# lbrndnr/LBAudioDetective

Measured on AMD Instinct MI355X. Metric: audio_seconds_fingerprinted_per_sec, higher is better.
Workload: dtype f32; 1 GPU; configs[1]: 100k synthetic 1 s @44.1 kHz mono clips, 1024-pt FFT, stride 64, fingerprint-only, input resident in HBM; one step = 13 passes over the batch; clips_per_gpu=100000, samples_per_clip=44100, window=1024, stride=64, bands=32, subfingerprints_per_clip=5, kernel_variant=0, parallelism=clips sharded x1, no collective

## Files before the change

### lbaudiodetective_amd/csrc/k_haar_select32.hip

```cpp
#include "internal.hpp"
#include "const_div.hpp"

#include <type_traits>

namespace lbad {
namespace {

constexpr uint32_t kCand = 128;
constexpr int kChunkDw = 20;


constexpr uint32_t kHistBuckets = 2048;

__device__ __forceinline__ uint32_t wave_prefix_sum(uint32_t x) {
    x += (uint32_t)__builtin_amdgcn_update_dpp(0, (int)x, 0x111 , 0xF, 0xF, false);
    x += (uint32_t)__builtin_amdgcn_update_dpp(0, (int)x, 0x112 , 0xF, 0xF, false);
    x += (uint32_t)__builtin_amdgcn_update_dpp(0, (int)x, 0x114 , 0xF, 0xF, false);
    x += (uint32_t)__builtin_amdgcn_update_dpp(0, (int)x, 0x118 , 0xF, 0xF, false);
    x += (uint32_t)__builtin_amdgcn_update_dpp(0, (int)x, 0x142 , 0xA, 0xF, false);
    x += (uint32_t)__builtin_amdgcn_update_dpp(0, (int)x, 0x143 , 0xC, 0xF, false);
    return x;
}

template <int WAVES>
__device__ __forceinline__ uint32_t slots_sum(const uint32_t* slot) {
    uint32_t c = 0;
#pragma unroll
    for (int w = 0; w < WAVES; ++w) c += slot[w];
    return c;
}

template <int WAVES>
__device__ __forceinline__ uint32_t block_sum(uint32_t v, uint32_t* s_red, int parity) {
#pragma unroll
    for (int off = 32; off > 0; off >>= 1) v += __shfl_xor(v, off, 64);
    uint32_t* slot = s_red + 8 * parity;
    if ((threadIdx.x & 63) == 0) slot[threadIdx.x >> 6] = v;
    __syncthreads();
    return slots_sum<WAVES>(slot);
}

constexpr uint32_t kLightLo = 0x25800000u;
typedef float f2 __attribute__((ext_vector_type(2)));

struct LightGuard {
    uint32_t lo_in = 0xFFFFFFFFu, lo_4 = 0xFFFFFFFFu;
    float hi = 0.0f;
    __device__ __forceinline__ void levels34(f2 a, f2 b, f2 c) {
        auto t = [](float x) { return (__float_as_uint(x) << 1) - 1u; };
        lo_4 = min(min(min(t(a.x), t(a.y)), min(t(b.x), t(b.y))), min(t(c.x), t(c.y)));
    }
    __device__ __forceinline__ bool bad(float s4) const {
        return lo_in < 2u * kLightLo - 1u || lo_4 < 2u * kFastDivLo - 1u || !(hi <= __uint_as_float(kFastDivHi)) || s4 != s4;
    }
};

template <bool FAST>
__device__ __forceinline__ float haar16_impl(const float (&in)[16], float (&d)[15], float root, float r_root,
                                             float root2, float r_root2, DivGuard& g) {
    float a[16];
#pragma unroll
    for (int i = 0; i < 16; i += 2) {
        if constexpr (FAST) {
            g.inputs(in[i], in[i + 1]);
            g.dividends(in[i], in[i + 1]);
        }
        a[i] = div_c<FAST>(in[i], root, r_root);
        a[i + 1] = div_c<FAST>(in[i + 1], root, r_root);
    }
    auto bfly = [&](float x, float y, float& sum, float& dif) {
        const float sp = __fadd_rn(x, y), sm = __fsub_rn(x, y);
        if constexpr (FAST) g.dividends(sp, sm);
        sum = div_c<FAST>(sp, root2, r_root2);
        dif = div_c<FAST>(sm, root2, r_root2);
    };
    float s1[8], s2[4], s3[2], s4;
#pragma unroll
    for (int i = 0; i < 8; ++i) bfly(a[2 * i], a[2 * i + 1], s1[i], d[i]);
#pragma unroll
    for (int i = 0; i < 4; ++i) bfly(s1[2 * i], s1[2 * i + 1], s2[i], d[8 + i]);
#pragma unroll
    for (int i = 0; i < 2; ++i) bfly(s2[2 * i], s2[2 * i + 1], s3[i], d[12 + i]);
    bfly(s3[0], s3[1], s4, d[14]);
    return s4;
}


struct DivConst {
    unsigned long long r, nd;
    __device__ __forceinline__ explicit DivConst(float d)
        : r(__builtin_amdgcn_readfirstlane(__float_as_uint(__fdiv_rn(1.0f, d)))),
          nd(__builtin_amdgcn_readfirstlane(__float_as_uint(-d))) {}
};

__device__ __forceinline__ void pk_prescale8(f2 (&x)[8], f2 (&q)[8], const DivConst& c) {
    asm("v_pk_mul_f32 %0, %8, %[r] op_sel_hi:[1,0]\n"
        "v_pk_mul_f32 %1, %9, %[r] op_sel_hi:[1,0]\n"
        "v_pk_mul_f32 %2, %10, %[r] op_sel_hi:[1,0]\n"
        "v_pk_mul_f32 %3, %11, %[r] op_sel_hi:[1,0]\n"
        "v_pk_mul_f32 %4, %12, %[r] op_sel_hi:[1,0]\n"
        "v_pk_mul_f32 %5, %13, %[r] op_sel_hi:[1,0]\n"
        "v_pk_mul_f32 %6, %14, %[r] op_sel_hi:[1,0]\n"
        "v_pk_mul_f32 %7, %15, %[r] op_sel_hi:[1,0]\n"
        "v_pk_fma_f32 %8, %0, %[nd], %8 op_sel_hi:[1,0,1]\n"
        "v_pk_fma_f32 %9, %1, %[nd], %9 op_sel_hi:[1,0,1]\n"
        "v_pk_fma_f32 %10, %2, %[nd], %10 op_sel_hi:[1,0,1]\n"
        "v_pk_fma_f32 %11, %3, %[nd], %11 op_sel_hi:[1,0,1]\n"
        "v_pk_fma_f32 %12, %4, %[nd], %12 op_sel_hi:[1,0,1]\n"
        "v_pk_fma_f32 %13, %5, %[nd], %13 op_sel_hi:[1,0,1]\n"
        "v_pk_fma_f32 %14, %6, %[nd], %14 op_sel_hi:[1,0,1]\n"
        "v_pk_fma_f32 %15, %7, %[nd], %15 op_sel_hi:[1,0,1]\n"
        "v_pk_fma_f32 %0, %8, %[r], %0 op_sel_hi:[1,0,1]\n"
        "v_pk_fma_f32 %1, %9, %[r], %1 op_sel_hi:[1,0,1]\n"
        "v_pk_fma_f32 %2, %10, %[r], %2 op_sel_hi:[1,0,1]\n"
        "v_pk_fma_f32 %3, %11, %[r], %3 op_sel_hi:[1,0,1]\n"
        "v_pk_fma_f32 %4, %12, %[r], %4 op_sel_hi:[1,0,1]\n"
        "v_pk_fma_f32 %5, %13, %[r], %5 op_sel_hi:[1,0,1]\n"
        "v_pk_fma_f32 %6, %14, %[r], %6 op_sel_hi:[1,0,1]\n"
        "v_pk_fma_f32 %7, %15, %[r], %7 op_sel_hi:[1,0,1]\n"
        "s_nop 0"
        : "=&v"(q[0]), "=&v"(q[1]), "=&v"(q[2]), "=&v"(q[3]), "=&v"(q[4]), "=&v"(q[5]), "=&v"(q[6]), "=&v"(q[7]),
          "+v"(x[0]), "+v"(x[1]), "+v"(x[2]), "+v"(x[3]), "+v"(x[4]), "+v"(x[5]), "+v"(x[6]), "+v"(x[7])
        : [r] "s"(c.r), [nd] "s"(c.nd));
}

__device__ __forceinline__ void pk_level1(f2 (&p)[8], f2 (&q)[8], const DivConst& c) {
    asm("v_pk_add_f32 %8, %8, %8 op_sel:[0,1] op_sel_hi:[0,1] neg_hi:[0,1]\n"
        "v_pk_add_f32 %9, %9, %9 op_sel:[0,1] op_sel_hi:[0,1] neg_hi:[0,1]\n"
        "v_pk_add_f32 %10, %10, %10 op_sel:[0,1] op_sel_hi:[0,1] neg_hi:[0,1]\n"
        "v_pk_add_f32 %11, %11, %11 op_sel:[0,1] op_sel_hi:[0,1] neg_hi:[0,1]\n"
        "v_pk_add_f32 %12, %12, %12 op_sel:[0,1] op_sel_hi:[0,1] neg_hi:[0,1]\n"
        "v_pk_add_f32 %13, %13, %13 op_sel:[0,1] op_sel_hi:[0,1] neg_hi:[0,1]\n"
        "v_pk_add_f32 %14, %14, %14 op_sel:[0,1] op_sel_hi:[0,1] neg_hi:[0,1]\n"
        "v_pk_add_f32 %15, %15, %15 op_sel:[0,1] op_sel_hi:[0,1] neg_hi:[0,1]\n"
        "v_pk_mul_f32 %0, %8, %[r] op_sel_hi:[1,0]\n"
        "v_pk_mul_f32 %1, %9, %[r] op_sel_hi:[1,0]\n"
        "v_pk_mul_f32 %2, %10, %[r] op_sel_hi:[1,0]\n"
        "v_pk_mul_f32 %3, %11, %[r] op_sel_hi:[1,0]\n"
        "v_pk_mul_f32 %4, %12, %[r] op_sel_hi:[1,0]\n"
        "v_pk_mul_f32 %5, %13, %[r] op_sel_hi:[1,0]\n"
        "v_pk_mul_f32 %6, %14, %[r] op_sel_hi:[1,0]\n"
        "v_pk_mul_f32 %7, %15, %[r] op_sel_hi:[1,0]\n"
        "v_pk_fma_f32 %8, %0, %[nd], %8 op_sel_hi:[1,0,1]\n"
        "v_pk_fma_f32 %9, %1, %[nd], %9 op_sel_hi:[1,0,1]\n"
        "v_pk_fma_f32 %10, %2, %[nd], %10 op_sel_hi:[1,0,1]\n"
        "v_pk_fma_f32 %11, %3, %[nd], %11 op_sel_hi:[1,0,1]\n"
        "v_pk_fma_f32 %12, %4, %[nd], %12 op_sel_hi:[1,0,1]\n"
        "v_pk_fma_f32 %13, %5, %[nd], %13 op_sel_hi:[1,0,1]\n"
        "v_pk_fma_f32 %14, %6, %[nd], %14 op_sel_hi:[1,0,1]\n"
        "v_pk_fma_f32 %15, %7, %[nd], %15 op_sel_hi:[1,0,1]\n"
        "v_pk_fma_f32 %0, %8, %[r], %0 op_sel_hi:[1,0,1]\n"
        "v_pk_fma_f32 %1, %9, %[r], %1 op_sel_hi:[1,0,1]\n"
        "v_pk_fma_f32 %2, %10, %[r], %2 op_sel_hi:[1,0,1]\n"
        "v_pk_fma_f32 %3, %11, %[r], %3 op_sel_hi:[1,0,1]\n"
        "v_pk_fma_f32 %4, %12, %[r], %4 op_sel_hi:[1,0,1]\n"
        "v_pk_fma_f32 %5, %13, %[r], %5 op_sel_hi:[1,0,1]\n"
        "v_pk_fma_f32 %6, %14, %[r], %6 op_sel_hi:[1,0,1]\n"
        "v_pk_fma_f32 %7, %15, %[r], %7 op_sel_hi:[1,0,1]\n"
        "s_nop 0"
        : "=&v"(q[0]), "=&v"(q[1]), "=&v"(q[2]), "=&v"(q[3]), "=&v"(q[4]), "=&v"(q[5]), "=&v"(q[6]), "=&v"(q[7]),
          "+v"(p[0]), "+v"(p[1]), "+v"(p[2]), "+v"(p[3]), "+v"(p[4]), "+v"(p[5]), "+v"(p[6]), "+v"(p[7])
        : [r] "s"(c.r), [nd] "s"(c.nd));
}

__device__ __forceinline__ void pk_level2(const f2 (&p)[8], f2 (&q)[4], const DivConst& c) {
    f2 t0, t1, t2, t3;
    asm("v_pk_add_f32 %4, %8, %9 op_sel:[0,0] op_sel_hi:[0,0] neg_hi:[0,1]\n"
        "v_pk_add_f32 %5, %10, %11 op_sel:[0,0] op_sel_hi:[0,0] neg_hi:[0,1]\n"
        "v_pk_add_f32 %6, %12, %13 op_sel:[0,0] op_sel_hi:[0,0] neg_hi:[0,1]\n"
        "v_pk_add_f32 %7, %14, %15 op_sel:[0,0] op_sel_hi:[0,0] neg_hi:[0,1]\n"
        "v_pk_mul_f32 %0, %4, %[r] op_sel_hi:[1,0]\n"
        "v_pk_mul_f32 %1, %5, %[r] op_sel_hi:[1,0]\n"
        "v_pk_mul_f32 %2, %6, %[r] op_sel_hi:[1,0]\n"
        "v_pk_mul_f32 %3, %7, %[r] op_sel_hi:[1,0]\n"
        "v_pk_fma_f32 %4, %0, %[nd], %4 op_sel_hi:[1,0,1]\n"
        "v_pk_fma_f32 %5, %1, %[nd], %5 op_sel_hi:[1,0,1]\n"
        "v_pk_fma_f32 %6, %2, %[nd], %6 op_sel_hi:[1,0,1]\n"
        "v_pk_fma_f32 %7, %3, %[nd], %7 op_sel_hi:[1,0,1]\n"
        "v_pk_fma_f32 %0, %4, %[r], %0 op_sel_hi:[1,0,1]\n"
        "v_pk_fma_f32 %1, %5, %[r], %1 op_sel_hi:[1,0,1]\n"
        "v_pk_fma_f32 %2, %6, %[r], %2 op_sel_hi:[1,0,1]\n"
        "v_pk_fma_f32 %3, %7, %[r], %3 op_sel_hi:[1,0,1]\n"
        "s_nop 0"
        : "=&v"(q[0]), "=&v"(q[1]), "=&v"(q[2]), "=&v"(q[3]), "=&v"(t0), "=&v"(t1), "=&v"(t2), "=&v"(t3)
        : "v"(p[0]), "v"(p[1]), "v"(p[2]), "v"(p[3]), "v"(p[4]), "v"(p[5]), "v"(p[6]), "v"(p[7]), [r] "s"(c.r), [nd] "s"(c.nd));
}

__device__ __forceinline__ void pk_level34(const f2 (&p)[4], f2 (&q3)[2], f2& q4, f2 (&s3)[2], f2& s4, const DivConst& c) {
    f2 e0, e1, e4;
    asm("v_pk_add_f32 %3, %9, %10 op_sel:[0,0] op_sel_hi:[0,0] neg_hi:[0,1]\n"
        "v_pk_add_f32 %4, %11, %12 op_sel:[0,0] op_sel_hi:[0,0] neg_hi:[0,1]\n"
        "v_pk_mul_f32 %0, %3, %[r] op_sel_hi:[1,0]\n"
        "v_pk_mul_f32 %1, %4, %[r] op_sel_hi:[1,0]\n"
        "v_pk_fma_f32 %6, %0, %[nd], %3 op_sel_hi:[1,0,1]\n"
        "v_pk_fma_f32 %7, %1, %[nd], %4 op_sel_hi:[1,0,1]\n"
        "v_pk_fma_f32 %0, %6, %[r], %0 op_sel_hi:[1,0,1]\n"
        "v_pk_fma_f32 %1, %7, %[r], %1 op_sel_hi:[1,0,1]\n"
        "s_nop 0\n"
        "v_pk_add_f32 %5, %0, %1 op_sel:[0,0] op_sel_hi:[0,0] neg_hi:[0,1]\n"
        "s_nop 0\n"
        "v_pk_mul_f32 %2, %5, %[r] op_sel_hi:[1,0]\n"
        "s_nop 0\n"
        "v_pk_fma_f32 %8, %2, %[nd], %5 op_sel_hi:[1,0,1]\n"
        "s_nop 0\n"
        "v_pk_fma_f32 %2, %8, %[r], %2 op_sel_hi:[1,0,1]\n"
        "s_nop 0"
        : "=&v"(q3[0]), "=&v"(q3[1]), "=&v"(q4), "=&v"(s3[0]), "=&v"(s3[1]), "=&v"(s4), "=&v"(e0), "=&v"(e1), "=&v"(e4)
        : "v"(p[0]), "v"(p[1]), "v"(p[2]), "v"(p[3]), [r] "s"(c.r), [nd] "s"(c.nd));
}

__device__ __forceinline__ float max3_abs(float m, float a, float b) {
    float o;
    asm("v_max3_f32 %0, %1, |%2|, |%3|" : "=v"(o) : "v"(m), "v"(a), "v"(b));
    return o;
}

template <typename Load>
__device__ __forceinline__ float haar16(Load load, float (&d)[15], float root, float root2, bool& fast) {
    const DivConst c_root(root), c_root2(root2);
    {
        f2 x[8], q[8], u[8], v2[4], w[2], z, s3[2], s4;
        {
            float in[16];
            load(in);
#pragma unroll
            for (int i = 0; i < 8; ++i) x[i] = f2{in[2 * i], in[2 * i + 1]};
        }
        LightGuard lg;
#pragma unroll
        for (int i = 0; i < 8; ++i) {
            lg.lo_in = min(lg.lo_in, min((__float_as_uint(x[i].x) << 1) - 1u, (__float_as_uint(x[i].y) << 1) - 1u));
            lg.hi = max3_abs(lg.hi, x[i].x, x[i].y);
        }
        pk_prescale8(x, q, c_root);
        pk_level1(q, u, c_root2);
        pk_level2(u, v2, c_root2);
        pk_level34(v2, w, z, s3, s4, c_root2);
        lg.levels34(s3[0], s3[1], s4);
        fast = !__any(lg.bad(z.x));
        if (fast) {
#pragma unroll
            for (int i = 0; i < 8; ++i) d[i] = u[i].y;
#pragma unroll
            for (int i = 0; i < 4; ++i) d[8 + i] = v2[i].y;
            d[12] = w[0].y; d[13] = w[1].y; d[14] = z.y;
            return z.x;
        }
    }
    asm volatile("" ::: "memory");
    float in[16];
    load(in);
    DivGuard g;
    float s4 = haar16_impl<true>(in, d, root, __fdiv_rn(1.0f, root), root2, __fdiv_rn(1.0f, root2), g);
    fast = !__any(g.bad());
    if (!fast) s4 = haar16_impl<false>(in, d, root, 0.0f, root2, 0.0f, g);
    return s4;
}

template <int M>
__device__ __forceinline__ float lane_xor(float x) {
    static_assert(M == 1 || M == 2 || M == 4, "lane distance");
    const int i = __float_as_int(x);
    if constexpr (M == 1) return __int_as_float(__builtin_amdgcn_mov_dpp(i, 0xB1, 0xF, 0xF, true));
    else if constexpr (M == 2) return __int_as_float(__builtin_amdgcn_mov_dpp(i, 0x4E, 0xF, 0xF, true));
    else return __int_as_float(__builtin_amdgcn_ds_swizzle(i, 0x101F));
}

template <bool FAST, int LANES, int M = 1>
__device__ __forceinline__ void cross_level_step(float& cur, float& fin, bool& done, int h, float root2, float r_root2, DivGuard& g) {
    if constexpr (M < LANES) {
        const float other = lane_xor<M>(cur);
        const bool upper = (h & M) != 0;
        const float lo = upper ? other : cur, hi = upper ? -cur : other;
        const float s = __fadd_rn(lo, hi);
        if constexpr (FAST) g.dividends(s, s);
        const float q = div_c<FAST>(s, root2, r_root2);
        if (!done && upper) { fin = q; done = true; }
        cur = q;
        cross_level_step<FAST, LANES, 2 * M>(cur, fin, done, h, root2, r_root2, g);
    }
}

template <bool FAST, int LANES>
__device__ __forceinline__ float cross_levels_impl(float cur, int h, float root2, float r_root2, DivGuard& g) {
    float fin = 0.0f;
    bool done = false;
    cross_level_step<FAST, LANES>(cur, fin, done, h, root2, r_root2, g);
    if (!done) fin = cur;
    return fin;
}

template <int LANES>
__device__ __forceinline__ float cross_levels(float cur, int h, float root2, bool fast) {
    if constexpr (LANES == 1) return cur;
    if (fast) {
        DivGuard g;
        const float fin = cross_levels_impl<true, LANES>(cur, h, root2, __fdiv_rn(1.0f, root2), g);
        if (!__any(g.bad())) return fin;
    }
    DivGuard g;
    return cross_levels_impl<false, LANES>(cur, h, root2, 0.0f, g);
}

struct SparseArgs {
    uint32_t left, n_cols;
    uint32_t row_dw;
    uint32_t pos_left;
    uint32_t pos_right[4];
    uint32_t cols[8];
    uint32_t rank[8];
};
constexpr int kSparseCols = 21;
__device__ __forceinline__ uint32_t byte_of(const uint32_t (&tbl)[8], uint32_t i) { return (tbl[i >> 2] >> (8u * (i & 3u))) & 0xFFu; }

constexpr uint32_t kRmask44k = 0xFFF5u;
typedef float f4u __attribute__((ext_vector_type(4), aligned(4)));
typedef float f3u __attribute__((ext_vector_type(3), aligned(4)));
typedef float f2u __attribute__((ext_vector_type(2), aligned(4)));

template <int COLS, bool SPARSE, uint32_t RMASK = 0u, bool HAS_LEFT = false>
__global__ __launch_bounds__(SPARSE ? 192 : COLS * 8, SPARSE ? 8 : COLS == 64 ? 6 : 7) void haar_select32_kernel(const float* __restrict__ frames, uint32_t keep,
                                                                          uint32_t subfp_len, uint32_t* __restrict__ packed,
                                                                          float* __restrict__ haar_out, const SparseArgs sp) {
    static_assert(!SPARSE || COLS == 32, "the sparse form is for 32 bands");
    constexpr int kCols = COLS;
    constexpr int kThreads = SPARSE ? 192 : COLS * 8;
    constexpr int kWavesPerWg = kThreads / 64;
    constexpr int H = COLS / 16;
    constexpr uint32_t kIdxBits = COLS == 16 ? 11 : COLS == 32 ? 12 : 13;
    __shared__ __attribute__((aligned(16))) float s_t[(SPARSE ? kSparseCols : kCols) * 8 * kChunkDw];
    __shared__ __attribute__((aligned(16))) unsigned long long s_cand[kCand];
    __shared__ uint32_t s_rank[kCand];
    __shared__ uint32_t s_red[16];
    __shared__ uint32_t s_ncand;
    __shared__ uint32_t s_bits[kPackedWords];
    __shared__ uint8_t s_pos[128];
    __shared__ uint32_t s_sel[4];
    static_assert(sizeof(s_t) >= kHistBuckets * sizeof(uint32_t), "the histogram lives in the transposed coefficients' LDS");

    const int t = threadIdx.x;
    const uint64_t frame = blockIdx.x;
    const float root2 = __fsqrt_rn(2.0f);
#ifdef LBAD_EXP_TIMELINE
    long long ts[8];
    int n_steps = 0;
#define STAMP(i) ts[i] = __builtin_readcyclecounter()
#define COUNT_STEP() ++n_steps
#else
#define STAMP(i)
#define COUNT_STEP()
#endif
    STAMP(0);

    float pre[16];
    float pre_left = 0.0f;
    auto fetch_row = [&](float (&a)[16], float& left_value) {
        if constexpr (SPARSE && RMASK != 0u) {
            constexpr int kRight = __builtin_popcount(RMASK), kRow = kRight + (HAS_LEFT ? 1 : 0);
            const bool mine = t < (int)kRowsPerFrame;
            const float* rowp = frames + frame * (kRowsPerFrame * kRow) + (mine ? t : 0) * kRow;
            float got[kRow + 3];
#pragma unroll
            for (int q = 0; q + 4 <= kRow; q += 4) {
                const f4u v = *reinterpret_cast<const f4u*>(rowp + q);
                got[q] = v.x; got[q + 1] = v.y; got[q + 2] = v.z; got[q + 3] = v.w;
            }
            constexpr int kDone = kRow & ~3;
            if constexpr (kRow - kDone == 3) {
                const f3u v = *reinterpret_cast<const f3u*>(rowp + kDone);
                got[kDone] = v.x; got[kDone + 1] = v.y; got[kDone + 2] = v.z;
            } else if constexpr (kRow - kDone == 2) {
                const f2u v = *reinterpret_cast<const f2u*>(rowp + kDone);
                got[kDone] = v.x; got[kDone + 1] = v.y;
            } else if constexpr (kRow - kDone == 1) {
                got[kDone] = rowp[kDone];
            }
#pragma unroll
            for (int jj = 0; jj < 16; ++jj)
                a[jj] = ((RMASK >> jj) & 1u) ? got[__builtin_popcount(RMASK & ((1u << jj) - 1u))] : 0.0f;
            left_value = HAS_LEFT ? got[kRight] : 0.0f;
        } else if constexpr (SPARSE) {
            const bool mine = t < (int)kRowsPerFrame;
            const float* rowp = frames + frame * (kRowsPerFrame * sp.row_dw) + (mine ? t : 0) * sp.row_dw;
            float got[16];
#pragma unroll
            for (int jj = 0; jj < 16; ++jj) {
                const uint32_t pos = (sp.pos_right[jj >> 2] >> (8 * (jj & 3))) & 0xFFu;
                got[jj] = rowp[pos != 0xFFu ? pos : 0u];
            }
            const float got_left = rowp[sp.left < 32u ? sp.pos_left : 0u];
#pragma unroll
            for (int jj = 0; jj < 16; ++jj) {
                const uint32_t pos = (sp.pos_right[jj >> 2] >> (8 * (jj & 3))) & 0xFFu;
                a[jj] = pos != 0xFFu ? got[jj] : 0.0f;
            }
            left_value = sp.left < 32u ? got_left : 0.0f;
        } else {
            const float4* src = reinterpret_cast<const float4*>(frames + frame * (kRowsPerFrame * kCols) + (t / H) * kCols + 16 * (t % H));
#pragma unroll
            for (int q = 0; q < 4; ++q) {
                const float4 v = src[q];
                a[4 * q] = v.x; a[4 * q + 1] = v.y; a[4 * q + 2] = v.z; a[4 * q + 3] = v.w;
            }
        }
    };
    fetch_row(pre, pre_left);
    bool first_read = true;

    if (t < (int)kPackedWords) s_bits[t] = 0;
    if (t < (int)kCand) s_rank[t] = 0;
    if (t == 0) s_ncand = 0;
    if (t < 128) {
        const int i = t >> 3, jj = t & 7;
        const int cross = (jj & 1) ? 4 + (jj >> 1) : (jj & 2) ? 2 + (jj >> 2) : (jj ? 1 : 0);
        s_pos[t] = (uint8_t)(i < 8 ? 64 + 8 * jj + i : i < 12 ? 32 + 4 * jj + (i - 8) : i < 14 ? 16 + 2 * jj + (i - 12) : i == 14 ? 8 + jj : cross);
    }
    for (int i = t; i < 2 * (int)kCand; i += kThreads)
        reinterpret_cast<uint32_t*>(s_cand)[i] = 0;

    if constexpr (SPARSE) {
        if (t < (int)kRowsPerFrame) {
            const int row = t;
            float d[15];
            auto load = [&](float (&a)[16]) {
                if (first_read) {
#pragma unroll
                    for (int jj = 0; jj < 16; ++jj) a[jj] = pre[jj];
                } else {
                    float again;
                    fetch_row(a, again);
                }
                first_read = false;
            };
            const float root = __fsqrt_rn(32.0f);
            bool fast;
            const float s4r = haar16(load, d, root, root2, fast);
            const float xl = pre_left;
            float det[4], s4l = 0.0f;
            auto chain = [&](auto fast_tag, DivGuard& g) {
                constexpr bool F = decltype(fast_tag)::value;
                const float r_root = F ? __fdiv_rn(1.0f, root) : 0.0f, r_root2 = F ? __fdiv_rn(1.0f, root2) : 0.0f;
                if constexpr (F) { g.inputs(xl, xl); g.dividends(xl, xl); }
                float a = div_c<F>(xl, root, r_root);
#pragma unroll
                for (int k = 0; k < 4; ++k) {
                    const bool odd = ((sp.left >> k) & 1u) != 0u;
                    const float sum_in = __fadd_rn(a, 0.0f);
                    if constexpr (F) g.dividends(sum_in, sum_in);
                    const float sum = div_c<F>(sum_in, root2, r_root2);
                    det[k] = odd ? -sum : sum;
                    a = sum;
                }
                s4l = a;
            };
            float avg = 0.0f, det5 = 0.0f;
            auto level5 = [&](auto fast_tag, DivGuard& g) {
                constexpr bool F = decltype(fast_tag)::value;
                const float r_root2 = F ? __fdiv_rn(1.0f, root2) : 0.0f;
                const float sp5 = __fadd_rn(s4l, s4r), sm5 = __fadd_rn(s4l, -s4r);
                if constexpr (F) g.dividends(sp5, sm5);
                avg = div_c<F>(sp5, root2, r_root2);
                det5 = div_c<F>(sm5, root2, r_root2);
            };
            {
                DivGuard g;
                chain(std::true_type{}, g);
                if (fast) level5(std::true_type{}, g);
                if (!fast || __any(g.bad())) {
                    chain(std::false_type{}, g);
                    level5(std::false_type{}, g);
                }
            }
            float* base = s_t + (row >> 4) * kChunkDw + (row & 15);
            auto put = [&](uint32_t pos, float value) {
                const uint32_t slot = byte_of(sp.rank, pos);
                if (slot != 0xFFu) base[slot * (8 * kChunkDw)] = value;
            };
#pragma unroll
            for (int i = 0; i < 8; ++i) put(24 + i, d[i]);
#pragma unroll
            for (int i = 0; i < 4; ++i) put(12 + i, d[8 + i]);
#pragma unroll
            for (int i = 0; i < 2; ++i) put(6 + i, d[12 + i]);
            put(3, d[14]);
            if (sp.left < 32u) {
                put(16 + (sp.left >> 1), det[0]);
                put(8 + (sp.left >> 2), det[1]);
                put(4 + (sp.left >> 3), det[2]);
                put(2, det[3]);
            }
            put(0, avg);
            put(1, det5);
        }
    } else
    {
        const int row = t / H, h = t % H;
        float d[15];
        auto load = [&](float (&a)[16]) {
            if (first_read) {
#pragma unroll
                for (int jj = 0; jj < 16; ++jj) a[jj] = pre[jj];
            } else {
                float unused;
                fetch_row(a, unused);
            }
            first_read = false;
        };
        bool fast;
        const float cur = haar16(load, d, __fsqrt_rn((float)kCols), root2, fast);
        const float fin = cross_levels<H>(cur, h, root2, fast);
        const int cross = H == 1 ? 0 : (h & 1) ? H / 2 + (h >> 1) : (h & 2) ? H / 4 + (h >> 2) : 0;
        float* base = s_t + (row >> 4) * kChunkDw + (row & 15);
#pragma unroll
        for (int i = 0; i < 8; ++i) base[(8 * H + 8 * h + i) * (8 * kChunkDw)] = d[i];
#pragma unroll
        for (int i = 0; i < 4; ++i) base[(4 * H + 4 * h + i) * (8 * kChunkDw)] = d[8 + i];
#pragma unroll
        for (int i = 0; i < 2; ++i) base[(2 * H + 2 * h + i) * (8 * kChunkDw)] = d[12 + i];
        base[(H + h) * (8 * kChunkDw)] = d[14];
        base[cross * (8 * kChunkDw)] = fin;
    }
    __syncthreads();
    STAMP(1);

    const bool live_thread = !SPARSE || (uint32_t)(t >> 3) < sp.n_cols;
    const bool live_wave = !SPARSE || (uint32_t)((t & ~63) >> 3) < sp.n_cols;
    const int cslot = SPARSE ? (live_thread ? t >> 3 : 0) : t >> 3;
    int col = t >> 3;
    if constexpr (SPARSE) col = (int)byte_of(sp.cols, (uint32_t)cslot);
    const int j = t & 7;
    float v[16];
    if (!live_wave) {
#pragma unroll
        for (int i = 0; i < 16; ++i) v[i] = 0.0f;
    } else {
        float d[15];
        const float4* src = reinterpret_cast<const float4*>(s_t + (cslot * 8 + j) * kChunkDw);
        auto load = [&](float (&a)[16]) {
#pragma unroll
            for (int q = 0; q < 4; ++q) {
                const float4 x = src[q];
                a[4 * q] = x.x; a[4 * q + 1] = x.y; a[4 * q + 2] = x.z; a[4 * q + 3] = x.w;
            }
        };
        bool fast;
        const float cur = haar16(load, d, __fsqrt_rn((float)kRowsPerFrame), root2, fast);
        const float fin = cross_levels<8>(cur, j, root2, fast);
#pragma unroll
        for (int i = 0; i < 8; ++i) v[i] = d[i];
#pragma unroll
        for (int i = 0; i < 4; ++i) v[8 + i] = d[8 + i];
        v[12] = d[12];
        v[13] = d[13];
        v[14] = d[14];
        v[15] = fin;
        if constexpr (SPARSE) {
            if (!live_thread) {
#pragma unroll
                for (int i = 0; i < 16; ++i) v[i] = 0.0f;
            }
        }
    }
    auto pos_of = [](int i, uint32_t jj) -> uint32_t {
        return i < 8 ? 64u + 8u * jj + (uint32_t)i : i < 12 ? 32u + 4u * jj + (uint32_t)(i - 8) : i < 14 ? 16u + 2u * jj + (uint32_t)(i - 12)
             : i == 14 ? 8u + jj : ((jj & 1u) ? 4u + (jj >> 1) : (jj & 2u) ? 2u + (jj >> 2) : (jj ? 1u : 0u));
    };
    auto opaque_j = [&]() -> uint32_t {
        uint32_t jj = (uint32_t)j;
        asm volatile("" : "+v"(jj));
        return jj;
    };
    if (haar_out && live_thread) {
        float* dst = haar_out + frame * (kRowsPerFrame * kCols);
        const uint32_t jj = opaque_j();
#pragma unroll
        for (int i = 0; i < 16; ++i) dst[pos_of(i, jj) * kCols + col] = v[i];
    }

    uint32_t key[16];
#pragma unroll
    for (int i = 0; i < 16; ++i) key[i] = __builtin_rotateleft32(__float_as_uint(v[i]), 1);

    STAMP(2);
    uint32_t lo = 0, hi = 0x80000000u, cnt_lo = kRowsPerFrame * kCols;
    uint32_t idx_bound = kRowsPerFrame * kCols;
    int parity = 0;
#ifndef LBAD_EXP_NO_HISTOGRAM
    {
        uint32_t* hist = reinterpret_cast<uint32_t*>(s_t);
        __syncthreads();
        for (int i = t; i < (int)(kHistBuckets / 4); i += kThreads) reinterpret_cast<uint4*>(hist)[i] = uint4{0u, 0u, 0u, 0u};
        __syncthreads();
        if (live_thread) {
            uint32_t any = 0;
#pragma unroll
            for (int i = 0; i < 16; ++i) any |= key[i];
            if (any > 1u) {
#pragma unroll
                for (int i = 0; i < 16; ++i) atomicAdd(&hist[key[i] >> 21], 1u);
            }
        }
        __syncthreads();
        if (t < 64) {
            const uint4* src = reinterpret_cast<const uint4*>(hist) + (kHistBuckets / 4 - 8 - 8 * t);
            uint32_t own = 0;
#pragma unroll
            for (int q = 0; q < 8; ++q) {
                const uint4 c = src[q];
                own += (c.x + c.y) + (c.z + c.w);
            }
            if (t == 63) own -= hist[0];
            const uint32_t incl = wave_prefix_sum(own), excl = incl - own;
            const unsigned long long m1 = __ballot(excl < keep && keep <= incl);
            uint32_t out_lo = 0, out_hi = 1u << 20, out_cnt = kRowsPerFrame * kCols;
            if (m1 != 0ull) {
                const int L = __ffsll((long long)m1) - 1;
                const uint32_t before = (uint32_t)__builtin_amdgcn_readlane((int)excl, L);
                const uint32_t top = kHistBuckets - 1u - 32u * (uint32_t)L;
                const uint32_t h = t < 32 ? hist[top - (uint32_t)t] : 0u;
                const uint32_t p = before + wave_prefix_sum(h);
                const unsigned long long m2 = __ballot(t < 32 && p - h < keep && keep <= p);
                const int J = __ffsll((long long)m2) - 1;
                const uint32_t b = top - (uint32_t)J;
                if (m2 != 0ull && b != 0u) {
                    out_lo = b << 20;
                    out_hi = (b + 1u) << 20;
                    out_cnt = (uint32_t)__builtin_amdgcn_readlane((int)p, J);
                }
            }
            if (t == 0) { s_sel[0] = out_lo; s_sel[1] = out_hi; s_sel[2] = out_cnt; }
        }
        __syncthreads();
        lo = s_sel[0];
        hi = s_sel[1];
        cnt_lo = s_sel[2];
    }
#endif
    while (cnt_lo > kCand && hi - lo > 1) {
        const uint32_t mid = lo + ((hi - lo) >> 1);
        uint32_t c = 0;
        if (live_wave) {
#pragma unroll
            for (int i = 0; i < 16; ++i) c += (uint32_t)__popcll(__ballot(key[i] >= (mid << 1)));
        }
        {
            uint32_t* slot = s_red + 8 * parity;
            if ((t & 63) == 0) slot[t >> 6] = c;
            __syncthreads();
            c = slots_sum<kWavesPerWg>(slot);
        }
        parity ^= 1;
        COUNT_STEP();
        if (c >= keep) { lo = mid; cnt_lo = c; } else { hi = mid; }
    }
    STAMP(3);
    const uint32_t lo2 = lo << 1;
    auto above = [&](uint32_t k) { return lo != 0x7FFFFFFFu && k >= lo2 + 2u; };
    auto tied = [&](uint32_t k) { return live_thread && k - lo2 < 2u; };
    if (cnt_lo > kCand) {
        uint32_t g = 0;
#pragma unroll
        for (int i = 0; i < 16; ++i) g += above(key[i]) ? 1u : 0u;
        g = block_sum<kWavesPerWg>(g, s_red, parity);
        parity ^= 1;
        const uint32_t jp = opaque_j();
        uint32_t ilo = 0, ihi = kRowsPerFrame * kCols;
        while (ilo < ihi) {
            const uint32_t im = ilo + ((ihi - ilo) >> 1);
            uint32_t c = 0;
#pragma unroll
            for (int i = 0; i < 16; ++i) c += (tied(key[i]) && pos_of(i, jp) * kCols + col < im) ? 1u : 0u;
            c = block_sum<kWavesPerWg>(c, s_red, parity);
            parity ^= 1;
            if (g + c >= keep) ihi = im; else ilo = im + 1;
        }
        idx_bound = ilo;
    }

    {
        const uint32_t origin = ((uint32_t)col << 7) | (uint32_t)j;
        typedef __attribute__((address_space(3))) void lds_void_t;
        uint32_t ncand_at = (uint32_t)(uintptr_t)(lds_void_t*)&s_ncand, one = 1u;
        asm volatile("" : "+v"(ncand_at), "+v"(one));
        auto gather = [&](auto selected) {
#ifdef LBAD_EXP_GATHER_BALLOT
#pragma unroll
            for (int h0 = 0; h0 < 16; h0 += 8) {
                unsigned long long mask[8];
                uint32_t wave_total = 0;
#pragma unroll
                for (int i = 0; i < 8; ++i) {
                    mask[i] = __ballot(selected(h0 + i));
                    wave_total += (uint32_t)__popcll(mask[i]);
                }
                if (wave_total == 0) continue;
                uint32_t base = 0;
                if ((t & 63) == 0) base = atomicAdd(&s_ncand, wave_total);
                base = __builtin_amdgcn_readfirstlane(base);
#pragma unroll
                for (int i = 0; i < 8; ++i) {
                    const unsigned long long m = mask[i];
                    if (selected(h0 + i)) {
                        const uint32_t at = base + __builtin_amdgcn_mbcnt_hi((uint32_t)(m >> 32), __builtin_amdgcn_mbcnt_lo((uint32_t)m, 0u));
                        s_cand[at] = ((unsigned long long)key[h0 + i] << 32) | (origin + (uint32_t)((h0 + i) << 3));
                    }
                    base += (uint32_t)__popcll(m);
                }
            }
#else
            uint32_t at[16];
#pragma unroll
            for (int i = 0; i < 16; ++i)
                if (selected(i)) asm volatile("ds_add_rtn_u32 %0, %1, %2" : "=v"(at[i]) : "v"(ncand_at), "v"(one) : "memory");
            asm volatile("s_waitcnt lgkmcnt(0)"
                         : "+v"(at[0]), "+v"(at[1]), "+v"(at[2]), "+v"(at[3]), "+v"(at[4]), "+v"(at[5]), "+v"(at[6]), "+v"(at[7]),
                           "+v"(at[8]), "+v"(at[9]), "+v"(at[10]), "+v"(at[11]), "+v"(at[12]), "+v"(at[13]), "+v"(at[14]), "+v"(at[15])
                         :: "memory");
#pragma unroll
            for (int i = 0; i < 16; ++i)
                if (selected(i)) s_cand[at[i]] = ((unsigned long long)key[i] << 32) | (origin + (uint32_t)(i << 3));
#endif
        };
        if (idx_bound == kRowsPerFrame * kCols) gather([&](int i) { return key[i] >= (lo << 1); });
        else {
            const uint32_t jg = opaque_j();
            gather([&](int i) { return above(key[i]) || (tied(key[i]) && pos_of(i, jg) * kCols + col < idx_bound); });
        }
    }
    __syncthreads();
    const uint32_t nc = s_ncand;
    if (t < (int)nc) {
        const unsigned long long raw = s_cand[t];
        const uint32_t k = (uint32_t)(raw >> 32), from = (uint32_t)raw;
        const uint32_t idx = (uint32_t)s_pos[from & 127u] * kCols + (from >> 7);
        const uint32_t sg = k - 2u < 0xFF000000u ? (k & 1u) + 1u : 0u;
        s_cand[t] = ((unsigned long long)(k & ~1u) << (kIdxBits + 1)) | ((unsigned long long)(((1u << kIdxBits) - 1u) - idx) << 2) | sg;
    }
    __syncthreads();
    STAMP(4);

    {
        constexpr uint32_t kGroup = kThreads == 192 ? 64 : 128;
        constexpr uint32_t kParts = kThreads / kGroup;
        constexpr uint32_t kPer = kCand / kGroup;
        const uint32_t part = t / kGroup, i0 = t % kGroup;
        const uint32_t nblk = (nc + 7) >> 3, pblk = (nblk + kParts - 1) / kParts;
        const uint32_t b0 = part * pblk < nblk ? part * pblk : nblk, b1 = b0 + pblk < nblk ? b0 + pblk : nblk;
        unsigned long long mine[kPer];
        uint32_t r[kPer];
#pragma unroll
        for (uint32_t k = 0; k < kPer; ++k) {
            const uint32_t i = i0 + k * kGroup;
            mine[k] = i < nc ? s_cand[i] : ~0ull;
            r[k] = 0;
        }
        for (uint32_t b = b0; b < b1; ++b) {
            const ulonglong2* src = reinterpret_cast<const ulonglong2*>(s_cand + 8 * b);
            const ulonglong2 c0 = src[0], c1 = src[1], c2 = src[2], c3 = src[3];
#pragma unroll
            for (uint32_t k = 0; k < kPer; ++k)
                r[k] += (c0.x > mine[k] ? 1u : 0u) + (c0.y > mine[k] ? 1u : 0u) + (c1.x > mine[k] ? 1u : 0u) + (c1.y > mine[k] ? 1u : 0u) +
                        (c2.x > mine[k] ? 1u : 0u) + (c2.y > mine[k] ? 1u : 0u) + (c3.x > mine[k] ? 1u : 0u) + (c3.y > mine[k] ? 1u : 0u);
        }
#pragma unroll
        for (uint32_t k = 0; k < kPer; ++k)
            if (r[k]) atomicAdd(&s_rank[i0 + k * kGroup], r[k]);
    }
    __syncthreads();
    if (t < (int)nc) {
        const uint32_t rank = s_rank[t];
        if (rank < keep) {
            const uint32_t sg = (uint32_t)s_cand[t] & 3u;
            const uint32_t b = 2 * rank;
            if (sg == 1u) atomicOr(&s_bits[b >> 5], 1u << (b & 31));
            else if (sg == 2u && b + 1 < subfp_len) atomicOr(&s_bits[(b + 1) >> 5], 1u << ((b + 1) & 31));
        }
    }
    __syncthreads();
    if (t < (int)kPackedWords) packed[frame * kPackedWords + t] = s_bits[t];
#ifdef LBAD_EXP_TIMELINE
    STAMP(5);
    if (haar_out && t == 0) {
        float* o = haar_out + frame * (kRowsPerFrame * kCols);
        for (int i = 1; i < 6; ++i) o[i - 1] = (float)(ts[i] - ts[i - 1]);
        o[5] = (float)n_steps;
        o[6] = (float)nc;
    }
#endif
}

}

bool haar_select32_supported(const Plan& p) {
    return (p.bands == 16 || p.bands == 32 || p.bands == 64) && p.keep <= kCand && p.keep >= 1;
}

hipError_t launch_haar_select32(const Plan& plan, const float* d_frames, uint64_t n_frames, uint32_t* d_packed,
                                float* d_haar_out, hipStream_t stream, bool compact) {
    if (n_frames == 0) return hipSuccess;
    if (n_frames > 0x7fffffffull) return hipErrorInvalidValue;
    SparseArgs sp = {};
    if (compact) {
        if (!plan.sparse.ok || plan.bands != 32) return hipErrorInvalidValue;
        if (plan.sparse.n_cols > (uint32_t)kSparseCols) return hipErrorInvalidValue;
        sp.left = plan.sparse.left;
        sp.n_cols = plan.sparse.n_cols;
        sp.row_dw = plan.sparse.n_stored;
        sp.pos_left = plan.sparse.pos_left;
        for (uint32_t j = 0; j < 16; ++j) sp.pos_right[j >> 2] |= (uint32_t)plan.sparse.pos_right[j] << (8u * (j & 3u));
        for (uint32_t i = 0; i < 8; ++i) sp.rank[i] = 0xFFFFFFFFu;
        for (uint32_t c = 0; c < 32; ++c) sp.cols[c >> 2] |= (uint32_t)plan.sparse.cols[c] << (8u * (c & 3u));
        for (uint32_t c = 0; c < plan.sparse.n_cols; ++c) {
            const uint32_t pos = plan.sparse.cols[c];
            sp.rank[pos >> 2] = (sp.rank[pos >> 2] & ~(0xFFu << (8u * (pos & 3u)))) | (c << (8u * (pos & 3u)));
        }
        uint32_t rmask = 0;
        for (uint32_t j = 0; j < 16; ++j)
            if (plan.sparse.pos_right[j] != 0xFF) rmask |= 1u << j;
        if (rmask == kRmask44k && plan.sparse.left < 32)
            hipLaunchKernelGGL((haar_select32_kernel<32, true, kRmask44k, true>), dim3((uint32_t)n_frames), dim3(192), 0, stream, d_frames,
                               plan.keep, plan.subfp_len, d_packed, d_haar_out, sp);
        else
            hipLaunchKernelGGL((haar_select32_kernel<32, true>), dim3((uint32_t)n_frames), dim3(192), 0, stream, d_frames, plan.keep,
                               plan.subfp_len, d_packed, d_haar_out, sp);
        return hipGetLastError();
    }
    if (plan.bands == 16)
        hipLaunchKernelGGL((haar_select32_kernel<16, false>), dim3((uint32_t)n_frames), dim3(128), 0, stream, d_frames, plan.keep,
                           plan.subfp_len, d_packed, d_haar_out, sp);
    else if (plan.bands == 64)
        hipLaunchKernelGGL((haar_select32_kernel<64, false>), dim3((uint32_t)n_frames), dim3(512), 0, stream, d_frames, plan.keep,
                           plan.subfp_len, d_packed, d_haar_out, sp);
    else
        hipLaunchKernelGGL((haar_select32_kernel<32, false>), dim3((uint32_t)n_frames), dim3(256), 0, stream, d_frames, plan.keep,
                           plan.subfp_len, d_packed, d_haar_out, sp);
    return hipGetLastError();
}

}
```

Baseline: 5.628 million audio-s/s.

## Bucket candidates by histogram bin so ranking compares only within each bucket

Turns the histogram into per-bucket cursors (exclusive prefix offsets) so the gather scatters candidates into bucket-sorted segments rather than appending through one shared counter. When no bucket exceeds a cap, each candidate's rank is its bucket's start plus a count over its own segment only, which replaces the all-pairs rank pass, the s_rank atomics and one barrier. s_rank is folded into the s_cand allocation and the upfront zeroing is dropped. The prefix walk adds serial wave work, and crowded frames still fall back to the all-pairs path.

```diff
diff --git a/lbaudiodetective_amd/csrc/k_haar_select32.hip b/lbaudiodetective_amd/csrc/k_haar_select32.hip
--- a/lbaudiodetective_amd/csrc/k_haar_select32.hip
+++ b/lbaudiodetective_amd/csrc/k_haar_select32.hip
@@ -11,6 +11,15 @@
 
 
 constexpr uint32_t kHistBuckets = 2048;
+
+constexpr uint32_t kSegCap = 64;
+constexpr uint32_t kCursorStep = 8;
+#if defined(LBAD_EXP_NO_HISTOGRAM) || defined(LBAD_EXP_GATHER_BALLOT)
+#define LBAD_ONE_CURSOR 1
+constexpr bool kBucketList = false;
+#else
+constexpr bool kBucketList = true;
+#endif
 
 __device__ __forceinline__ uint32_t wave_prefix_sum(uint32_t x) {
     x += (uint32_t)__builtin_amdgcn_update_dpp(0, (int)x, 0x111 , 0xF, 0xF, false);
@@ -329,10 +338,12 @@
     constexpr int H = COLS / 16;
     constexpr uint32_t kIdxBits = COLS == 16 ? 11 : COLS == 32 ? 12 : 13;
     __shared__ __attribute__((aligned(16))) float s_t[(SPARSE ? kSparseCols : kCols) * 8 * kChunkDw];
-    __shared__ __attribute__((aligned(16))) unsigned long long s_cand[kCand];
-    __shared__ uint32_t s_rank[kCand];
+    __shared__ __attribute__((aligned(16))) unsigned long long s_cand[kCand + kCand / 2];
+    uint32_t* const s_rank = reinterpret_cast<uint32_t*>(s_cand + kCand);
     __shared__ uint32_t s_red[16];
+#ifdef LBAD_ONE_CURSOR
     __shared__ uint32_t s_ncand;
+#endif
     __shared__ uint32_t s_bits[kPackedWords];
     __shared__ uint8_t s_pos[128];
     __shared__ uint32_t s_sel[4];
@@ -408,16 +419,14 @@
     bool first_read = true;
 
     if (t < (int)kPackedWords) s_bits[t] = 0;
-    if (t < (int)kCand) s_rank[t] = 0;
+#ifdef LBAD_ONE_CURSOR
     if (t == 0) s_ncand = 0;
+#endif
     if (t < 128) {
         const int i = t >> 3, jj = t & 7;
         const int cross = (jj & 1) ? 4 + (jj >> 1) : (jj & 2) ? 2 + (jj >> 2) : (jj ? 1 : 0);
         s_pos[t] = (uint8_t)(i < 8 ? 64 + 8 * jj + i : i < 12 ? 32 + 4 * jj + (i - 8) : i < 14 ? 16 + 2 * jj + (i - 12) : i == 14 ? 8 + jj : cross);
     }
-    for (int i = t; i < 2 * (int)kCand; i += kThreads)
-        reinterpret_cast<uint32_t*>(s_cand)[i] = 0;
-
     if constexpr (SPARSE) {
         if (t < (int)kRowsPerFrame) {
             const int row = t;
@@ -585,9 +594,10 @@
     uint32_t lo = 0, hi = 0x80000000u, cnt_lo = kRowsPerFrame * kCols;
     uint32_t idx_bound = kRowsPerFrame * kCols;
     int parity = 0;
+    bool all_pairs = true;
+    uint32_t* const hist = reinterpret_cast<uint32_t*>(s_t);
 #ifndef LBAD_EXP_NO_HISTOGRAM
     {
-        uint32_t* hist = reinterpret_cast<uint32_t*>(s_t);
         __syncthreads();
         for (int i = t; i < (int)(kHistBuckets / 4); i += kThreads) reinterpret_cast<uint4*>(hist)[i] = uint4{0u, 0u, 0u, 0u};
         __syncthreads();
@@ -613,6 +623,7 @@
             const uint32_t incl = wave_prefix_sum(own), excl = incl - own;
             const unsigned long long m1 = __ballot(excl < keep && keep <= incl);
             uint32_t out_lo = 0, out_hi = 1u << 20, out_cnt = kRowsPerFrame * kCols;
+            int thr_bucket = 0;
             if (m1 != 0ull) {
                 const int L = __ffsll((long long)m1) - 1;
                 const uint32_t before = (uint32_t)__builtin_amdgcn_readlane((int)excl, L);
@@ -626,14 +637,33 @@
                     out_lo = b << 20;
                     out_hi = (b + 1u) << 20;
                     out_cnt = (uint32_t)__builtin_amdgcn_readlane((int)p, J);
+                    thr_bucket = (int)b;
                 }
             }
-            if (t == 0) { s_sel[0] = out_lo; s_sel[1] = out_hi; s_sel[2] = out_cnt; }
+            uint32_t crowded = 1u;
+            if constexpr (kBucketList) {
+                const unsigned long long held = __ballot(own != 0u);
+                const int l0 = held != 0ull ? __ffsll((long long)held) - 1 : 63;
+                uint32_t above = (uint32_t)__builtin_amdgcn_readlane((int)excl, l0);
+                unsigned long long wide = 0ull;
+                for (int base = (int)kHistBuckets - 1 - 32 * l0; base >= thr_bucket; base -= 64) {
+                    const int bkt = base - t;
+                    const uint32_t h = bkt >= 0 ? hist[bkt] : 0u;
+                    const uint32_t upto = wave_prefix_sum(h);
+                    const uint32_t start = (above + upto - h) * kCursorStep;
+                    if (bkt >= 0) hist[bkt] = start + (start << 16);
+                    wide |= __ballot(bkt >= thr_bucket && h > kSegCap);
+                    above += (uint32_t)__builtin_amdgcn_readlane((int)upto, 63);
+                }
+                crowded = out_cnt > kCand || wide != 0ull ? 1u : 0u;
+            }
+            if (t == 0) { s_sel[0] = out_lo; s_sel[1] = out_hi; s_sel[2] = out_cnt; s_sel[3] = crowded; }
         }
         __syncthreads();
         lo = s_sel[0];
         hi = s_sel[1];
         cnt_lo = s_sel[2];
+        all_pairs = s_sel[3] != 0u;
     }
 #endif
     while (cnt_lo > kCand && hi - lo > 1) {
@@ -680,8 +710,18 @@
     {
         const uint32_t origin = ((uint32_t)col << 7) | (uint32_t)j;
         typedef __attribute__((address_space(3))) void lds_void_t;
-        uint32_t ncand_at = (uint32_t)(uintptr_t)(lds_void_t*)&s_ncand, one = 1u;
-        asm volatile("" : "+v"(ncand_at), "+v"(one));
+#ifdef LBAD_ONE_CURSOR
+        uint32_t step = 1u;
+        uint32_t ncand_at = (uint32_t)(uintptr_t)(lds_void_t*)&s_ncand;
+        asm volatile("" : "+v"(ncand_at));
+        auto cursor_of = [&](uint32_t) { return ncand_at; };
+        auto slot_of = [&](uint32_t got) { return &s_cand[got]; };
+#else
+        uint32_t step = kCursorStep;
+        auto cursor_of = [&](uint32_t k) { return (uint32_t)(uintptr_t)(lds_void_t*)&hist[k >> 21]; };
+        auto slot_of = [&](uint32_t got) { return reinterpret_cast<unsigned long long*>(reinterpret_cast<char*>(s_cand) + (got & 0xFFFFu)); };
+#endif
+        asm volatile("" : "+v"(step));
         auto gather = [&](auto selected) {
 #ifdef LBAD_EXP_GATHER_BALLOT
 #pragma unroll
@@ -711,14 +751,14 @@
             uint32_t at[16];
 #pragma unroll
             for (int i = 0; i < 16; ++i)
-                if (selected(i)) asm volatile("ds_add_rtn_u32 %0, %1, %2" : "=v"(at[i]) : "v"(ncand_at), "v"(one) : "memory");
+                if (selected(i)) asm volatile("ds_add_rtn_u32 %0, %1, %2" : "=v"(at[i]) : "v"(cursor_of(key[i])), "v"(step) : "memory");
             asm volatile("s_waitcnt lgkmcnt(0)"
                          : "+v"(at[0]), "+v"(at[1]), "+v"(at[2]), "+v"(at[3]), "+v"(at[4]), "+v"(at[5]), "+v"(at[6]), "+v"(at[7]),
                            "+v"(at[8]), "+v"(at[9]), "+v"(at[10]), "+v"(at[11]), "+v"(at[12]), "+v"(at[13]), "+v"(at[14]), "+v"(at[15])
                          :: "memory");
 #pragma unroll
             for (int i = 0; i < 16; ++i)
-                if (selected(i)) s_cand[at[i]] = ((unsigned long long)key[i] << 32) | (origin + (uint32_t)(i << 3));
+                if (selected(i)) *slot_of(at[i]) = ((unsigned long long)key[i] << 32) | (origin + (uint32_t)(i << 3));
 #endif
         };
         if (idx_bound == kRowsPerFrame * kCols) gather([&](int i) { return key[i] >= (lo << 1); });
@@ -728,18 +768,47 @@
         }
     }
     __syncthreads();
+#ifdef LBAD_ONE_CURSOR
     const uint32_t nc = s_ncand;
+#else
+    const uint32_t nc = (hist[lo >> 20] & 0xFFFFu) / kCursorStep;
+#endif
+    unsigned long long own = 0;
+    uint32_t seg = 0;
     if (t < (int)nc) {
         const unsigned long long raw = s_cand[t];
         const uint32_t k = (uint32_t)(raw >> 32), from = (uint32_t)raw;
+        if constexpr (kBucketList) seg = hist[k >> 21];
         const uint32_t idx = (uint32_t)s_pos[from & 127u] * kCols + (from >> 7);
         const uint32_t sg = k - 2u < 0xFF000000u ? (k & 1u) + 1u : 0u;
-        s_cand[t] = ((unsigned long long)(k & ~1u) << (kIdxBits + 1)) | ((unsigned long long)(((1u << kIdxBits) - 1u) - idx) << 2) | sg;
-    }
-    __syncthreads();
-    STAMP(4);
-
-    {
+        own = ((unsigned long long)(k & ~1u) << (kIdxBits + 1)) | ((unsigned long long)(((1u << kIdxBits) - 1u) - idx) << 2) | sg;
+        s_cand[t] = own;
+    }
+    auto emit = [&](uint32_t rank, uint32_t sg) {
+        if (rank < keep) {
+            const uint32_t b = 2 * rank;
+            if (sg == 1u) atomicOr(&s_bits[b >> 5], 1u << (b & 31));
+            else if (sg == 2u && b + 1 < subfp_len) atomicOr(&s_bits[(b + 1) >> 5], 1u << ((b + 1) & 31));
+        }
+    };
+    if (!all_pairs) {
+        if (t < 3) s_cand[nc + t] = 0;
+        __syncthreads();
+        STAMP(4);
+        if (t < (int)nc) {
+            const uint32_t end = (seg & 0xFFFFu) / kCursorStep;
+            uint32_t rank = (seg >> 16) / kCursorStep;
+            for (uint32_t i = rank; i < end; i += 4) {
+                const unsigned long long c0 = s_cand[i], c1 = s_cand[i + 1], c2 = s_cand[i + 2], c3 = s_cand[i + 3];
+                rank += (c0 > own ? 1u : 0u) + (c1 > own ? 1u : 0u) + (c2 > own ? 1u : 0u) + (c3 > own ? 1u : 0u);
+            }
+            emit(rank, (uint32_t)own & 3u);
+        }
+    } else {
+        if (t < (int)kCand) s_rank[t] = 0;
+        if (t >= (int)nc && t < (int)((nc + 7u) & ~7u)) s_cand[t] = 0;
+        __syncthreads();
+        STAMP(4);
         constexpr uint32_t kGroup = kThreads == 192 ? 64 : 128;
         constexpr uint32_t kParts = kThreads / kGroup;
         constexpr uint32_t kPer = kCand / kGroup;
@@ -765,16 +834,8 @@
 #pragma unroll
         for (uint32_t k = 0; k < kPer; ++k)
             if (r[k]) atomicAdd(&s_rank[i0 + k * kGroup], r[k]);
-    }
-    __syncthreads();
-    if (t < (int)nc) {
-        const uint32_t rank = s_rank[t];
-        if (rank < keep) {
-            const uint32_t sg = (uint32_t)s_cand[t] & 3u;
-            const uint32_t b = 2 * rank;
-            if (sg == 1u) atomicOr(&s_bits[b >> 5], 1u << (b & 31));
-            else if (sg == 2u && b + 1 < subfp_len) atomicOr(&s_bits[(b + 1) >> 5], 1u << ((b + 1) & 31));
-        }
+        __syncthreads();
+        if (t < (int)nc) emit(s_rank[t], (uint32_t)own & 3u);
     }
     __syncthreads();
     if (t < (int)kPackedWords) packed[frame * kPackedWords + t] = s_bits[t];
```

Measured after the change: 5.706 million audio-s/s (median of 6 runs). +1.4%, better.
